# JoHof/lungmask

Hardware: NVIDIA H100
Metric: CT slices/sec @256x256 (R231) (higher is better)
Workload: dtype f16x3 (fp32-class: every fp32 value is an fp16 hi + scaled fp16 lo pair, 3 exact products per MAC, fp32 accumulate)

## Files before the change

lungmask_b200/csrc/conv_tc.cu:

```cuda
#include <atomic>
#include <stdio.h>
#include "conv_tc.cuh"
#include "sm90_ptx.cuh"

namespace lm {
namespace {

constexpr int BM = 128, BK = kBK, TILE_H = 16, TILE_W = 8;
constexpr int ROW_BYTES = 128;
constexpr int HALO_W = TILE_W + 2, HALO_H = TILE_H + 2;
constexpr int A_PLANE_BYTES_3x3 = HALO_W * HALO_H * ROW_BYTES;
constexpr int A_PLANE_BYTES_1x1 = BM * ROW_BYTES;
constexpr int A_BUF_BYTES = 2 * A_PLANE_BYTES_3x3;
constexpr int NUM_A_BUFS = 2;
constexpr int NUM_THREADS = 384;
constexpr int NUM_CONSUMER_WARPS = 8;
constexpr int MAX_CLASSES = 8;
constexpr int REGS_PRODUCER = 40, REGS_CONSUMER = 232;

template <int BN>
struct Cfg {
  static constexpr int B_PLANE_BYTES = BN * ROW_BYTES;
  static constexpr int STAGE_BYTES = 2 * B_PLANE_BYTES;
  static constexpr int STAGES = (BN == 64) ? 6 : 4;
  static constexpr int NUM_BARS = 2 * STAGES + 2 * NUM_A_BUFS;
  static constexpr int OFF_B = NUM_A_BUFS * A_BUF_BYTES;
  static constexpr int OFF_BARS = OFF_B + STAGES * STAGE_BYTES;
  static constexpr int OFF_HEAD = OFF_BARS + NUM_BARS * 8;
  static constexpr int DYN_SMEM = OFF_HEAD + ((BN == 64) ? (MAX_CLASSES * 64 + MAX_CLASSES) * 4 : 0);
  static_assert(DYN_SMEM <= 232448, "shared-memory budget (227 KB per CTA)");
};

struct TileCoord {
  int n, y0, x0, n0;
};

__device__ __forceinline__ TileCoord decode_tile(int tile, int n_tiles, int tiles_x, int tiles_img, int BN) {
  TileCoord t;
  const int mt = tile / n_tiles;
  t.n0 = (tile - mt * n_tiles) * BN;
  t.n = mt / tiles_img;
  const int r = mt - t.n * tiles_img;
  const int ty = r / tiles_x;
  t.y0 = ty * TILE_H;
  t.x0 = (r - ty * tiles_x) * TILE_W;
  return t;
}

template <int MC>
struct WorkItems {
  int first, step, total, n_tiles;
  uint32_t rank;
  __device__ WorkItems(int total_tiles, int n_tiles_) : n_tiles(n_tiles_) {
    rank = (MC > 1) ? cluster_ctarank() : 0u;
    first = (int)blockIdx.x / MC;
    step = (int)gridDim.x / MC;
    total = total_tiles / MC;
  }
  __device__ int tile(int item) const {
    if (MC == 1) return item;
    const int mtp = item / n_tiles;
    return (MC * mtp + (int)rank) * n_tiles + (item - mtp * n_tiles);
  }
};

__device__ __forceinline__ void store_split_pair(op_t* dst, size_t plane_stride, float a, float b) {
#if LM_OPERAND_F16
  uint32_t hi, lo;
  split_f16x2(a, b, hi, lo);
  *reinterpret_cast<uint32_t*>(dst) = hi;
  *reinterpret_cast<uint32_t*>(dst + plane_stride) = lo;
#else
  float ha, la, hb, lb;
  split_tf32(a, ha, la);
  split_tf32(b, hb, lb);
  *reinterpret_cast<float2*>(dst) = make_float2(ha, hb);
  *reinterpret_cast<float2*>(dst + plane_stride) = make_float2(la, lb);
#endif
}

__device__ __forceinline__ float2 ldg2_or_zero(const float* p, int c) {
  return p ? __ldg(reinterpret_cast<const float2*>(p + c)) : make_float2(0.f, 0.f);
}

template <int BN, int TAPS, int MC>
__device__ __forceinline__ void conv_consumer(const ConvParams& p, uint32_t smem_a, uint32_t smem_b, uint32_t full0,
                                              uint32_t empty0, uint32_t afull0, uint32_t aempty0, const float* s_head_w,
                                              const float* s_head_b) {
  using C = Cfg<BN>;
  constexpr int NA = BN / 2;
  constexpr int STAGES = C::STAGES;
  constexpr int PATCH_W = (TAPS == 9) ? HALO_W : TILE_W;
  constexpr uint32_t A_PLANE = (uint32_t)((TAPS == 9) ? A_PLANE_BYTES_3x3 : A_PLANE_BYTES_1x1);
  constexpr uint32_t SBO_A = PATCH_W * ROW_BYTES;
  const int tid = threadIdx.x - 128;
  const int half = tid >> 7, wq = (tid >> 5) & 3, lane = tid & 31;
  const int g = lane >> 2, qd = lane & 3;
  const int tiles_x = p.W / TILE_W, tiles_img = tiles_x * (p.H / TILE_H);
  const int n_tiles = p.Cout / BN;
  const int total_tiles = p.N * tiles_img * n_tiles;
  const int num_cb = (p.C0 + p.C1) / BK;
  const int num_kb = num_cb * TAPS, chunk_kb = p.chunk_kb;
  const uint32_t a_half = (uint32_t)(8 * half * PATCH_W * ROW_BYTES);

  const WorkItems<MC> items(total_tiles, n_tiles);
  float S[NA], P[NA], Q[NA];
  uint32_t s = 0, ph = 0, ab = 0, aph = 0;
  auto release = [&](uint32_t st, int a) {
    __syncwarp();
    if (lane == 0) {
      mbar_arrive(empty0 + 8 * st);
      if (MC > 1) mbar_arrive_cluster(empty0 + 8 * st, items.rank ^ 1u);
      if (a >= 0) mbar_arrive(aempty0 + 8 * a);
    }
  };
  auto mma_one = [&](float (&D)[NA], uint64_t da, uint64_t db, int acc) {
    if constexpr (BN == 128) wgmma_n128(D, da, db, acc); else wgmma_n64(D, da, db, acc);
  };

  for (int item = items.first; item < items.total; item += items.step) {
    const TileCoord t = decode_tile(items.tile(item), n_tiles, tiles_x, tiles_img, BN);
#pragma unroll
    for (int i = 0; i < NA; ++i) { S[i] = 0.f; Q[i] = 0.f; }
    for (int kb0 = 0; kb0 < num_kb; kb0 += chunk_kb) {
      const int kb1 = min(kb0 + chunk_kb, num_kb);
      uint32_t pend_s = 0;
      int pend_a = -1;
      for (int kb = kb0; kb < kb1; ++kb) {
        const int tap = (TAPS == 9) ? kb % 9 : 0;
        if (tap == 0) mbar_spin(afull0 + 8 * ab, aph);
        const uint32_t a_tap = smem_a + ab * (uint32_t)A_BUF_BYTES + a_half + (uint32_t)(((tap / 3) * PATCH_W + (tap % 3)) * ROW_BYTES);
        const uint32_t b_st = smem_b + s * (uint32_t)C::STAGE_BYTES;
        mbar_spin(full0 + 8 * s, ph);
        wgmma_fence();
#pragma unroll
        for (int k = 0; k < ROW_BYTES / 32; ++k) {
          const uint64_t ah = make_desc_sw128(a_tap + 32 * k, SBO_A), al = make_desc_sw128(a_tap + A_PLANE + 32 * k, SBO_A);
          const uint64_t bh = make_desc_sw128(b_st + 32 * k, 1024), bl = make_desc_sw128(b_st + C::B_PLANE_BYTES + 32 * k, 1024);
          mma_one(P, ah, bh, k != 0 || kb != kb0);
          mma_one(Q, ah, bl, 1);
          mma_one(Q, al, bh, 1);
        }
        wgmma_commit();
        if (kb > kb0) {
          wgmma_wait<1>();
          release(pend_s, pend_a);
        }
        pend_s = s;
        pend_a = (tap == TAPS - 1) ? (int)ab : -1;
        if (++s == STAGES) { s = 0; ph ^= 1u; }
        if (tap == TAPS - 1 && ++ab == NUM_A_BUFS) { ab = 0; aph ^= 1u; }
      }
      wgmma_wait<0>();
      release(pend_s, pend_a);
#pragma unroll
      for (int i = 0; i < NA; ++i) S[i] += P[i];
    }
#pragma unroll
    for (int i = 0; i < NA; ++i) S[i] += Q[i] * kLoUnscale;

    const float unscale = p.in_unscale;
    const int y = t.y0 + 8 * half + 2 * wq, x = t.x0 + g;
    const int c0 = t.n0 + 2 * qd;
    if (p.mode == kModeLinear) {
      float* out = static_cast<float*>(p.out);
#pragma unroll
      for (int j = 0; j < BN / 8; ++j) {
        const int c = c0 + 8 * j;
        const float2 b = ldg2_or_zero(p.bias, c);
#pragma unroll
        for (int r = 0; r < 2; ++r)
          *reinterpret_cast<float2*>(out + (((size_t)t.n * p.H + y + r) * p.W + x) * p.Cout + c) =
              make_float2(__fmaf_rn(S[4 * j + 2 * r], unscale, b.x), __fmaf_rn(S[4 * j + 2 * r + 1], unscale, b.y));
      }
      continue;
    }
    const float cscale = (p.mode == kModeHead) ? 1.f : p.out_scale;
#pragma unroll
    for (int j = 0; j < BN / 8; ++j) {
      const int c = c0 + 8 * j;
      const float2 b = ldg2_or_zero(p.bias, c), sc = ldg2_or_zero(p.scale, c), sh = ldg2_or_zero(p.shift, c);
      const float s0 = sc.x * cscale, s1 = sc.y * cscale, h0 = sh.x * cscale, h1 = sh.y * cscale;
#pragma unroll
      for (int r = 0; r < 2; ++r) {
        float& v0 = S[4 * j + 2 * r];
        float& v1 = S[4 * j + 2 * r + 1];
        v0 = __fadd_rn(__fmul_rn(fmaxf(__fmaf_rn(v0, unscale, b.x), 0.f), s0), h0);
        v1 = __fadd_rn(__fmul_rn(fmaxf(__fmaf_rn(v1, unscale, b.y), 0.f), s1), h1);
      }
    }
    if (BN == 64 && p.mode == kModeHead) {
      float lg[2][MAX_CLASSES];
#pragma unroll
      for (int k = 0; k < MAX_CLASSES; ++k) {
        float d0 = 0.f, d1 = 0.f;
        if (k < p.K) {
#pragma unroll
          for (int j = 0; j < BN / 8; ++j) {
#pragma unroll
            for (int e = 0; e < 2; ++e) {
              const float w = s_head_w[k * 64 + 8 * j + 2 * qd + e];
              d0 = fmaf(w, S[4 * j + e], d0);
              d1 = fmaf(w, S[4 * j + 2 + e], d1);
            }
          }
        }
        d0 += __shfl_xor_sync(0xffffffffu, d0, 1);
        d1 += __shfl_xor_sync(0xffffffffu, d1, 1);
        d0 += __shfl_xor_sync(0xffffffffu, d0, 2);
        d1 += __shfl_xor_sync(0xffffffffu, d1, 2);
        lg[0][k] = (k < p.K) ? d0 + s_head_b[k] : -INFINITY;
        lg[1][k] = (k < p.K) ? d1 + s_head_b[k] : -INFINITY;
      }
      if (qd == 0) {
#pragma unroll
        for (int r = 0; r < 2; ++r) {
          float mx = -INFINITY;
#pragma unroll
          for (int k = 0; k < MAX_CLASSES; ++k) mx = fmaxf(mx, lg[r][k]);
          float se = 0.f;
#pragma unroll
          for (int k = 0; k < MAX_CLASSES; ++k) if (k < p.K) se += expf(lg[r][k] - mx);
          const float lse = logf(se);
          int best = 0;
          float bestv = -INFINITY;
#pragma unroll
          for (int k = 0; k < MAX_CLASSES; ++k) {
            if (k < p.K) {
              const float sc = (lg[r][k] - mx) - lse;
              if (sc > bestv) { bestv = sc; best = k; }
              if (p.scores) p.scores[(((size_t)t.n * p.K + k) * p.H + y + r) * p.W + x] = sc;
            }
          }
          p.labels[((size_t)t.n * p.H + y + r) * p.W + x] = (uint8_t)best;
        }
      }
      continue;
    }
#if LM_OPERAND_F16
    {
      bool ovf = false;
#pragma unroll
      for (int i = 0; i < NA; ++i) ovf |= !(fabsf(S[i]) <= kOpMax);
      if (__any_sync(0xffffffffu, ovf) && lane == 0 && p.range_flag) *p.range_flag = 1;
    }
#endif
    {
      const size_t plane = (size_t)p.H * p.W * p.Cout;
      op_t* img = static_cast<op_t*>(p.out) + (size_t)t.n * 2 * plane;
#pragma unroll
      for (int j = 0; j < BN / 8; ++j)
#pragma unroll
        for (int r = 0; r < 2; ++r)
          store_split_pair(img + ((size_t)(y + r) * p.W + x) * p.Cout + c0 + 8 * j, plane, S[4 * j + 2 * r], S[4 * j + 2 * r + 1]);
    }
    if (p.mode == kModeReluBnPool) {
      const int Hp = p.H / 2, Wp = p.W / 2;
      const size_t plane = (size_t)Hp * Wp * p.Cout;
      op_t* img = static_cast<op_t*>(p.out_pool) + (size_t)t.n * 2 * plane + ((size_t)(y >> 1) * Wp + (x >> 1)) * p.Cout + c0;
#pragma unroll
      for (int j = 0; j < BN / 8; ++j) {
        float pv[2];
#pragma unroll
        for (int e = 0; e < 2; ++e) {
          const float top = S[4 * j + e] + __shfl_xor_sync(0xffffffffu, S[4 * j + e], 4);
          const float bot = S[4 * j + 2 + e] + __shfl_xor_sync(0xffffffffu, S[4 * j + 2 + e], 4);
          pv[e] = (top + bot) * 0.25f;
        }
        if ((g & 1) == 0) store_split_pair(img + 8 * j, plane, pv[0], pv[1]);
      }
    }
  }
}

template <int BN, int MC>
__global__ void __launch_bounds__(NUM_THREADS, 1)
conv_tc_kernel(const __grid_constant__ CUtensorMap tmA0, const __grid_constant__ CUtensorMap tmA1,
               const __grid_constant__ CUtensorMap tmB, const __grid_constant__ CUtensorMap tmBX, const ConvParams p) {
  using C = Cfg<BN>;
  constexpr int STAGES = C::STAGES;
  extern __shared__ __align__(1024) uint8_t smem[];
  uint64_t* bars = reinterpret_cast<uint64_t*>(smem + C::OFF_BARS);
  float* s_head_w = reinterpret_cast<float*>(smem + C::OFF_HEAD);
  float* s_head_b = s_head_w + MAX_CLASSES * 64;
  const uint32_t full0 = smem_u32(&bars[0]), empty0 = full0 + 8 * STAGES;
  const uint32_t afull0 = full0 + 16 * STAGES, aempty0 = afull0 + 8 * NUM_A_BUFS;
  const uint32_t smem_a = smem_u32(smem), smem_b = smem_a + C::OFF_B;
  const int warp = threadIdx.x >> 5;

  if (threadIdx.x == 0) {
    for (int s = 0; s < STAGES; ++s) { mbar_init(full0 + 8 * s, 1); mbar_init(empty0 + 8 * s, MC * NUM_CONSUMER_WARPS); }
    for (int s = 0; s < NUM_A_BUFS; ++s) { mbar_init(afull0 + 8 * s, 1); mbar_init(aempty0 + 8 * s, NUM_CONSUMER_WARPS); }
    fence_mbar_init();
    tma_prefetch_desc(&tmA0); tma_prefetch_desc(&tmA1); tma_prefetch_desc(MC > 1 ? &tmBX : &tmB);
  }
  if (BN == 64 && p.mode == kModeHead) {
    for (int i = threadIdx.x; i < p.K * 64; i += NUM_THREADS) s_head_w[i] = p.head_w[i];
    if (threadIdx.x < p.K) s_head_b[threadIdx.x] = p.head_b[threadIdx.x];
  }
  __syncthreads();
  if (MC > 1) cluster_sync_all();

  if (warp >= 4) {
    setmaxnreg_inc<REGS_CONSUMER>();
    if (p.taps == 9) conv_consumer<BN, 9, MC>(p, smem_a, smem_b, full0, empty0, afull0, aempty0, s_head_w, s_head_b);
    else conv_consumer<BN, 1, MC>(p, smem_a, smem_b, full0, empty0, afull0, aempty0, s_head_w, s_head_b);
  } else {
    setmaxnreg_dec<REGS_PRODUCER>();
    if (warp == 0) {
      const int tiles_x = p.W / TILE_W, tiles_img = tiles_x * (p.H / TILE_H);
      const int n_tiles = p.Cout / BN;
      const WorkItems<MC> items(p.N * tiles_img * n_tiles, n_tiles);
      const int taps = p.taps, halo = taps == 9 ? 1 : 0;
      const int num_cb = (p.C0 + p.C1) / BK;
      const uint32_t a_tx = 2u * (uint32_t)(taps == 9 ? A_PLANE_BYTES_3x3 : A_PLANE_BYTES_1x1);
      uint32_t s = 0, ph = 0, ab = 0, aph = 0;
      for (int item = items.first; item < items.total; item += items.step) {
        const TileCoord t = decode_tile(items.tile(item), n_tiles, tiles_x, tiles_img, BN);
        int c = 0;
        for (int cb = 0; cb < num_cb; ++cb, c += BK) {
          mbar_wait_inline(aempty0 + 8 * ab, aph ^ 1);
          if (elect_one()) {
            mbar_arrive_expect_tx(afull0 + 8 * ab, a_tx);
            const uint32_t dst = smem_a + ab * A_BUF_BYTES;
            if (c < p.C0) tma_load_5d(dst, &tmA0, afull0 + 8 * ab, c, t.x0 - halo, t.y0 - halo, 0, t.n);
            else          tma_load_5d(dst, &tmA1, afull0 + 8 * ab, c - p.C0, t.x0 - halo, t.y0 - halo, 0, t.n);
          }
          __syncwarp();
          if (++ab == NUM_A_BUFS) { ab = 0; aph ^= 1; }
          for (int tap = 0; tap < taps; ++tap) {
            mbar_wait_inline(empty0 + 8 * s, ph ^ 1);
            if (elect_one()) {
              mbar_arrive_expect_tx(full0 + 8 * s, C::STAGE_BYTES);
              if (MC > 1)
                tma_load_4d_mcast(smem_b + s * C::STAGE_BYTES + items.rank * (uint32_t)C::B_PLANE_BYTES, &tmBX, full0 + 8 * s, c, t.n0,
                                  tap, (int)items.rank, (uint16_t)((1u << MC) - 1u));
              else
                tma_load_4d(smem_b + s * C::STAGE_BYTES, &tmB, full0 + 8 * s, c, t.n0, tap, 0);
            }
            __syncwarp();
            if (++s == STAGES) { s = 0; ph ^= 1; }
          }
        }
      }
    }
  }
  if (MC > 1) cluster_sync_all();
}

typedef CUresult (*EncodeTiledFn)(CUtensorMap*, CUtensorMapDataType, cuuint32_t, void*, const cuuint64_t*,
                                  const cuuint64_t*, const cuuint32_t*, const cuuint32_t*,
                                  CUtensorMapInterleave, CUtensorMapSwizzle, CUtensorMapL2promotion,
                                  CUtensorMapFloatOOBfill);

EncodeTiledFn get_encode_fn() {
  static EncodeTiledFn fn = nullptr;
  if (!fn) {
    void* f = nullptr;
    cudaDriverEntryPointQueryResult qres;
    if (cudaGetDriverEntryPoint("cuTensorMapEncodeTiled", &f, cudaEnableDefault, &qres) != cudaSuccess) return nullptr;
    fn = reinterpret_cast<EncodeTiledFn>(f);
  }
  return fn;
}

#if LM_OPERAND_F16
constexpr CUtensorMapDataType kOpType = CU_TENSOR_MAP_DATA_TYPE_FLOAT16;
#else
constexpr CUtensorMapDataType kOpType = CU_TENSOR_MAP_DATA_TYPE_FLOAT32;
#endif

int encode(CUtensorMap* m, CUtensorMapDataType dtype, const void* base, int rank, const cuuint64_t* dims,
           const cuuint64_t* strides, const cuuint32_t* box) {
  EncodeTiledFn fn = get_encode_fn();
  if (!fn) return -1;
  cuuint32_t es[5] = {1, 1, 1, 1, 1};
  CUresult r = fn(m, dtype, (cuuint32_t)rank, const_cast<void*>(base), dims, strides, box,
                  es, CU_TENSOR_MAP_INTERLEAVE_NONE, CU_TENSOR_MAP_SWIZZLE_128B,
                  CU_TENSOR_MAP_L2_PROMOTION_L2_256B, CU_TENSOR_MAP_FLOAT_OOB_FILL_NONE);
  return r == CUDA_SUCCESS ? 0 : (int)r;
}

int make_act_map(CUtensorMap* m, const void* base, int n_cap, int H, int W, int Cch, int taps) {
  const cuuint64_t E = kOpBytes;
  cuuint64_t dims[5] = {(cuuint64_t)Cch, (cuuint64_t)W, (cuuint64_t)H, 2, (cuuint64_t)n_cap};
  cuuint64_t strides[4] = {(cuuint64_t)Cch * E, (cuuint64_t)W * Cch * E, (cuuint64_t)H * W * Cch * E,
                           (cuuint64_t)2 * H * W * Cch * E};
  const cuuint32_t halo = taps == 9 ? 2 : 0;
  cuuint32_t box[5] = {BK, TILE_W + halo, TILE_H + halo, 2, 1};
  return encode(m, kOpType, base, 5, dims, strides, box);
}

}

int make_conv_maps(ConvMaps* maps, const void* src0, const void* src1, const void* weights,
                   const ConvParams& p, int n_capacity) {
  const cuuint64_t E = kOpBytes;
  if (p.H % TILE_H || p.W % TILE_W || p.C0 % BK || p.C1 % BK || (p.taps != 1 && p.taps != 9)) return -2;
  const int BN = conv_tile_n(p);
  if (p.Cout % BN) return -3;
  int r = make_act_map(&maps->a0, src0, n_capacity, p.H, p.W, p.C0, p.taps);
  if (r) return r;
  r = (p.C1 > 0) ? make_act_map(&maps->a1, src1, n_capacity, p.H, p.W, p.C1, p.taps)
                 : make_act_map(&maps->a1, src0, n_capacity, p.H, p.W, p.C0, p.taps);
  if (r) return r;
  const int Cin = p.C0 + p.C1;
  cuuint64_t dims[4] = {(cuuint64_t)Cin, (cuuint64_t)p.Cout, (cuuint64_t)p.taps, 2};
  cuuint64_t strides[3] = {(cuuint64_t)Cin * E, (cuuint64_t)p.Cout * Cin * E, (cuuint64_t)p.taps * p.Cout * Cin * E};
  cuuint32_t box[4] = {BK, (cuuint32_t)BN, 1, 2}, box_x[4] = {BK, (cuuint32_t)BN, 1, 1};
  r = encode(&maps->b, kOpType, weights, 4, dims, strides, box);
  return r ? r : encode(&maps->bx, kOpType, weights, 4, dims, strides, box_x);
}


template <int BN, int MC>
static int launch_impl(const ConvMaps& maps, const ConvParams& p, int num_sms, cudaStream_t stream) {
  static std::atomic<unsigned long long> attr_set_mask{0ull};
  int dev = 0;
  if (cudaGetDevice(&dev) != cudaSuccess || dev < 0 || dev >= 64) return -9;
  if (!((attr_set_mask.load(std::memory_order_acquire) >> dev) & 1ull)) {
    cudaError_t e = cudaFuncSetAttribute(conv_tc_kernel<BN, MC>, cudaFuncAttributeMaxDynamicSharedMemorySize, Cfg<BN>::DYN_SMEM);
    if (e != cudaSuccess) return (int)e;
    attr_set_mask.fetch_or(1ull << dev, std::memory_order_release);
  }
  const int total = p.N * (p.H / TILE_H) * (p.W / TILE_W) * (p.Cout / BN);
  const int groups = total / MC, sm_groups = num_sms / MC;
  cudaLaunchConfig_t cfg = {};
  cfg.gridDim = dim3((unsigned)(MC * (groups < sm_groups ? groups : sm_groups)), 1, 1);
  cfg.blockDim = dim3(NUM_THREADS, 1, 1);
  cfg.dynamicSmemBytes = Cfg<BN>::DYN_SMEM;
  cfg.stream = stream;
  cudaLaunchAttribute attr[1];
  attr[0].id = cudaLaunchAttributeClusterDimension;
  attr[0].val.clusterDim.x = MC; attr[0].val.clusterDim.y = 1; attr[0].val.clusterDim.z = 1;
  cfg.attrs = attr;
  cfg.numAttrs = 1;
  cudaError_t e = cudaLaunchKernelEx(&cfg, conv_tc_kernel<BN, MC>, maps.a0, maps.a1, maps.b, maps.bx, p);
  return (int)(e != cudaSuccess ? e : cudaGetLastError());
}

int conv_tc_prepare() {
  cudaError_t e = cudaFuncSetAttribute(conv_tc_kernel<128, 1>, cudaFuncAttributeMaxDynamicSharedMemorySize, Cfg<128>::DYN_SMEM);
  if (e == cudaSuccess) e = cudaFuncSetAttribute(conv_tc_kernel<64, 1>, cudaFuncAttributeMaxDynamicSharedMemorySize, Cfg<64>::DYN_SMEM);
  if (e == cudaSuccess) e = cudaFuncSetAttribute(conv_tc_kernel<128, 2>, cudaFuncAttributeMaxDynamicSharedMemorySize, Cfg<128>::DYN_SMEM);
  if (e == cudaSuccess) e = cudaFuncSetAttribute(conv_tc_kernel<64, 2>, cudaFuncAttributeMaxDynamicSharedMemorySize, Cfg<64>::DYN_SMEM);
  return (int)e;
}

int launch_conv_tc(const ConvMaps& maps, const ConvParams& p, int num_sms, cudaStream_t stream) {
  if (p.mode == kModeHead && (p.Cout != 64 || p.K > MAX_CLASSES)) return -4;
  if (p.chunk_kb < 1) return -5;
  if (p.weight_mcast == 2)
    return conv_tile_n(p) == 128 ? launch_impl<128, 2>(maps, p, num_sms, stream) : launch_impl<64, 2>(maps, p, num_sms, stream);
  return conv_tile_n(p) == 128 ? launch_impl<128, 1>(maps, p, num_sms, stream) : launch_impl<64, 1>(maps, p, num_sms, stream);
}

}
```

Before: 1392.

## Overlap next tile's first WGMMAs with epilogue; vectorize stores via quad transpose

The consumer now issues the first one or two k-blocks of the next tile's MMAs before running the current tile's epilogue, so tensor-core work overlaps the epilogue's stores and arithmetic. This uses extra accumulator registers (P2 for BN=64), and the release and fold bookkeeping becomes more intricate. Epilogue stores are also regrouped with an intra-quad shuffle transpose so each thread writes 16-byte vectors instead of 4- or 8-byte pieces, cutting store instruction count at the cost of extra shuffles. Head-mode BN=64 and 1x1 layers keep the old path.

New measurement: 1473 (median of 6 runs). 1.06x the previous value.

```diff
diff --git a/lungmask_b200/csrc/conv_tc.cu b/lungmask_b200/csrc/conv_tc.cu
--- a/lungmask_b200/csrc/conv_tc.cu
+++ b/lungmask_b200/csrc/conv_tc.cu
@@ -64,18 +64,57 @@
   }
 };
 
-__device__ __forceinline__ void store_split_pair(op_t* dst, size_t plane_stride, float a, float b) {
+__device__ __forceinline__ void quad_transpose(uint32_t (&x)[4], int qd) {
+#pragma unroll
+  for (int m = 2; m >= 1; m >>= 1) {
+    const bool up = (qd & m) != 0;
+#pragma unroll
+    for (int k = 0; k < 4; ++k) {
+      if (k & m) continue;
+      const uint32_t recv = __shfl_xor_sync(0xffffffffu, up ? x[k] : x[k ^ m], m);
+      x[k] = up ? recv : x[k];
+      x[k ^ m] = up ? x[k ^ m] : recv;
+    }
+  }
+}
+__device__ __forceinline__ void quad_transpose(float2 (&v)[4], int qd) {
+  uint32_t a[4], b[4];
+#pragma unroll
+  for (int k = 0; k < 4; ++k) { a[k] = __float_as_uint(v[k].x); b[k] = __float_as_uint(v[k].y); }
+  quad_transpose(a, qd);
+  quad_transpose(b, qd);
+#pragma unroll
+  for (int k = 0; k < 4; ++k) v[k] = make_float2(__uint_as_float(a[k]), __uint_as_float(b[k]));
+}
+
+__device__ __forceinline__ void store_split8(op_t* dst, size_t plane_stride, const float2 (&v)[4], int qd, bool pred) {
 #if LM_OPERAND_F16
-  uint32_t hi, lo;
-  split_f16x2(a, b, hi, lo);
-  *reinterpret_cast<uint32_t*>(dst) = hi;
-  *reinterpret_cast<uint32_t*>(dst + plane_stride) = lo;
+  uint32_t hi[4], lo[4];
+#pragma unroll
+  for (int k = 0; k < 4; ++k) split_f16x2(v[k].x, v[k].y, hi[k], lo[k]);
+  quad_transpose(hi, qd);
+  quad_transpose(lo, qd);
+  if (pred) {
+    *reinterpret_cast<uint4*>(dst) = make_uint4(hi[0], hi[1], hi[2], hi[3]);
+    *reinterpret_cast<uint4*>(dst + plane_stride) = make_uint4(lo[0], lo[1], lo[2], lo[3]);
+  }
 #else
-  float ha, la, hb, lb;
-  split_tf32(a, ha, la);
-  split_tf32(b, hb, lb);
-  *reinterpret_cast<float2*>(dst) = make_float2(ha, hb);
-  *reinterpret_cast<float2*>(dst + plane_stride) = make_float2(la, lb);
+  float2 h[4], l[4];
+#pragma unroll
+  for (int k = 0; k < 4; ++k) {
+    split_tf32(v[k].x, h[k].x, l[k].x);
+    split_tf32(v[k].y, h[k].y, l[k].y);
+  }
+  quad_transpose(h, qd);
+  quad_transpose(l, qd);
+  if (pred) {
+    float4* dh = reinterpret_cast<float4*>(dst);
+    float4* dl = reinterpret_cast<float4*>(dst + plane_stride);
+    dh[0] = make_float4(h[0].x, h[0].y, h[1].x, h[1].y);
+    dh[1] = make_float4(h[2].x, h[2].y, h[3].x, h[3].y);
+    dl[0] = make_float4(l[0].x, l[0].y, l[1].x, l[1].y);
+    dl[1] = make_float4(l[2].x, l[2].y, l[3].x, l[3].y);
+  }
 #endif
 }
 
@@ -83,7 +122,7 @@
   return p ? __ldg(reinterpret_cast<const float2*>(p + c)) : make_float2(0.f, 0.f);
 }
 
-template <int BN, int TAPS, int MC>
+template <int BN, int TAPS, int MC, bool LOOKAHEAD>
 __device__ __forceinline__ void conv_consumer(const ConvParams& p, uint32_t smem_a, uint32_t smem_b, uint32_t full0,
                                               uint32_t empty0, uint32_t afull0, uint32_t aempty0, const float* s_head_w,
                                               const float* s_head_b) {
@@ -102,9 +141,14 @@
   const int num_cb = (p.C0 + p.C1) / BK;
   const int num_kb = num_cb * TAPS, chunk_kb = p.chunk_kb;
   const uint32_t a_half = (uint32_t)(8 * half * PATCH_W * ROW_BYTES);
+  static_assert(!LOOKAHEAD || TAPS == 9, "look-ahead: 3x3 layers only");
+  const int la = !LOOKAHEAD ? 0 : (BN == 64 || chunk_kb >= 2) ? 2 : 1;
+  const bool la_split = BN == 64 && chunk_kb == 1 && la == 2;
+  const bool la_fold = la > 0 && (la_split || la % chunk_kb == 0 || la == num_kb);
 
   const WorkItems<MC> items(total_tiles, n_tiles);
   float S[NA], P[NA], Q[NA];
+  float P2[(BN == 64) ? NA : 1];
   uint32_t s = 0, ph = 0, ab = 0, aph = 0;
   auto release = [&](uint32_t st, int a) {
     __syncwarp();
@@ -117,61 +161,115 @@
   auto mma_one = [&](float (&D)[NA], uint64_t da, uint64_t db, int acc) {
     if constexpr (BN == 128) wgmma_n128(D, da, db, acc); else wgmma_n64(D, da, db, acc);
   };
-
-  for (int item = items.first; item < items.total; item += items.step) {
-    const TileCoord t = decode_tile(items.tile(item), n_tiles, tiles_x, tiles_img, BN);
-#pragma unroll
-    for (int i = 0; i < NA; ++i) { S[i] = 0.f; Q[i] = 0.f; }
-    for (int kb0 = 0; kb0 < num_kb; kb0 += chunk_kb) {
-      const int kb1 = min(kb0 + chunk_kb, num_kb);
+  auto issue_kb = [&](float (&D)[NA], int kb, bool hh_restart) -> int {
+    const int tap = (TAPS == 9) ? kb % 9 : 0;
+    if (tap == 0) mbar_spin(afull0 + 8 * ab, aph);
+    const uint32_t a_tap = smem_a + ab * (uint32_t)A_BUF_BYTES + a_half + (uint32_t)(((tap / 3) * PATCH_W + (tap % 3)) * ROW_BYTES);
+    const uint32_t b_st = smem_b + s * (uint32_t)C::STAGE_BYTES;
+    mbar_spin(full0 + 8 * s, ph);
+    wgmma_fence();
+#pragma unroll
+    for (int k = 0; k < ROW_BYTES / 32; ++k) {
+      const uint64_t ah = make_desc_sw128(a_tap + 32 * k, SBO_A), al = make_desc_sw128(a_tap + A_PLANE + 32 * k, SBO_A);
+      const uint64_t bh = make_desc_sw128(b_st + 32 * k, 1024), bl = make_desc_sw128(b_st + C::B_PLANE_BYTES + 32 * k, 1024);
+      mma_one(D, ah, bh, k != 0 || !hh_restart);
+      mma_one(Q, ah, bl, 1);
+      mma_one(Q, al, bh, 1);
+    }
+    wgmma_commit();
+    const int a = (tap == TAPS - 1) ? (int)ab : -1;
+    if (++s == STAGES) { s = 0; ph ^= 1u; }
+    if (tap == TAPS - 1 && ++ab == NUM_A_BUFS) { ab = 0; aph ^= 1u; }
+    return a;
+  };
+  uint32_t la_s = 0;
+  auto issue_lookahead = [&]() {
+    if constexpr (LOOKAHEAD) {
+#pragma unroll
+      for (int i = 0; i < NA; ++i) Q[i] = 0.f;
+      la_s = s;
+      issue_kb(P, 0, true);
+      if (la_split) {
+        if constexpr (BN == 64) issue_kb(P2, 1, true);
+      } else if (la > 1) {
+        issue_kb(P, 1, false);
+      }
+    }
+  };
+
+  int item = items.first;
+  if (item < items.total) issue_lookahead();
+  for (; item < items.total; item += items.step) {
+    wgmma_wait<0>();
+    if constexpr (LOOKAHEAD) {
+      release(la_s, -1);
+      if (la > 1) release(la_s + 1 == STAGES ? 0 : la_s + 1, -1);
+    } else {
+#pragma unroll
+      for (int i = 0; i < NA; ++i) Q[i] = 0.f;
+    }
+#pragma unroll
+    for (int i = 0; i < NA; ++i) S[i] = 0.f;
+    if (la_fold) {
+#pragma unroll
+      for (int i = 0; i < NA; ++i) S[i] += P[i];
+      if constexpr (BN == 64) {
+        if (la_split) {
+#pragma unroll
+          for (int i = 0; i < NA; ++i) S[i] += P2[i];
+        }
+      }
+    }
+    for (int kb0 = la; kb0 < num_kb;) {
+      const int kb1 = min((kb0 / chunk_kb + 1) * chunk_kb, num_kb);
+      const bool restart = kb0 % chunk_kb == 0;
       uint32_t pend_s = 0;
       int pend_a = -1;
       for (int kb = kb0; kb < kb1; ++kb) {
-        const int tap = (TAPS == 9) ? kb % 9 : 0;
-        if (tap == 0) mbar_spin(afull0 + 8 * ab, aph);
-        const uint32_t a_tap = smem_a + ab * (uint32_t)A_BUF_BYTES + a_half + (uint32_t)(((tap / 3) * PATCH_W + (tap % 3)) * ROW_BYTES);
-        const uint32_t b_st = smem_b + s * (uint32_t)C::STAGE_BYTES;
-        mbar_spin(full0 + 8 * s, ph);
-        wgmma_fence();
-#pragma unroll
-        for (int k = 0; k < ROW_BYTES / 32; ++k) {
-          const uint64_t ah = make_desc_sw128(a_tap + 32 * k, SBO_A), al = make_desc_sw128(a_tap + A_PLANE + 32 * k, SBO_A);
-          const uint64_t bh = make_desc_sw128(b_st + 32 * k, 1024), bl = make_desc_sw128(b_st + C::B_PLANE_BYTES + 32 * k, 1024);
-          mma_one(P, ah, bh, k != 0 || kb != kb0);
-          mma_one(Q, ah, bl, 1);
-          mma_one(Q, al, bh, 1);
-        }
-        wgmma_commit();
+        const uint32_t st = s;
+        const int a = issue_kb(P, kb, restart && kb == kb0);
         if (kb > kb0) {
           wgmma_wait<1>();
           release(pend_s, pend_a);
         }
-        pend_s = s;
-        pend_a = (tap == TAPS - 1) ? (int)ab : -1;
-        if (++s == STAGES) { s = 0; ph ^= 1u; }
-        if (tap == TAPS - 1 && ++ab == NUM_A_BUFS) { ab = 0; aph ^= 1u; }
+        pend_s = st;
+        pend_a = a;
       }
       wgmma_wait<0>();
       release(pend_s, pend_a);
 #pragma unroll
       for (int i = 0; i < NA; ++i) S[i] += P[i];
+      kb0 = kb1;
     }
 #pragma unroll
     for (int i = 0; i < NA; ++i) S[i] += Q[i] * kLoUnscale;
 
+    if (item + items.step < items.total) issue_lookahead();
+    const TileCoord tc = decode_tile(items.tile(item), n_tiles, tiles_x, tiles_img, BN);
+
     const float unscale = p.in_unscale;
-    const int y = t.y0 + 8 * half + 2 * wq, x = t.x0 + g;
-    const int c0 = t.n0 + 2 * qd;
+    const int y = tc.y0 + 8 * half + 2 * wq, x = tc.x0 + g;
+    const int c0 = tc.n0 + 2 * qd;
     if (p.mode == kModeLinear) {
-      float* out = static_cast<float*>(p.out);
-#pragma unroll
-      for (int j = 0; j < BN / 8; ++j) {
-        const int c = c0 + 8 * j;
-        const float2 b = ldg2_or_zero(p.bias, c);
-#pragma unroll
-        for (int r = 0; r < 2; ++r)
-          *reinterpret_cast<float2*>(out + (((size_t)t.n * p.H + y + r) * p.W + x) * p.Cout + c) =
-              make_float2(__fmaf_rn(S[4 * j + 2 * r], unscale, b.x), __fmaf_rn(S[4 * j + 2 * r + 1], unscale, b.y));
+      float* out = static_cast<float*>(p.out) + ((size_t)tc.n * p.H * p.W + x) * p.Cout + tc.n0 + 8 * qd;
+#pragma unroll
+      for (int m = 0; m < BN / 32; ++m) {
+        float2 b[4];
+#pragma unroll
+        for (int k = 0; k < 4; ++k) b[k] = ldg2_or_zero(p.bias, c0 + 8 * (4 * m + k));
+#pragma unroll
+        for (int r = 0; r < 2; ++r) {
+          float2 v[4];
+#pragma unroll
+          for (int k = 0; k < 4; ++k) {
+            const int j = 4 * m + k;
+            v[k] = make_float2(__fmaf_rn(S[4 * j + 2 * r], unscale, b[k].x), __fmaf_rn(S[4 * j + 2 * r + 1], unscale, b[k].y));
+          }
+          quad_transpose(v, qd);
+          float4* dst = reinterpret_cast<float4*>(out + (size_t)(y + r) * p.W * p.Cout + 32 * m);
+          dst[0] = make_float4(v[0].x, v[0].y, v[1].x, v[1].y);
+          dst[1] = make_float4(v[2].x, v[2].y, v[3].x, v[3].y);
+        }
       }
       continue;
     }
@@ -229,10 +327,10 @@
             if (k < p.K) {
               const float sc = (lg[r][k] - mx) - lse;
               if (sc > bestv) { bestv = sc; best = k; }
-              if (p.scores) p.scores[(((size_t)t.n * p.K + k) * p.H + y + r) * p.W + x] = sc;
+              if (p.scores) p.scores[(((size_t)tc.n * p.K + k) * p.H + y + r) * p.W + x] = sc;
             }
           }
-          p.labels[((size_t)t.n * p.H + y + r) * p.W + x] = (uint8_t)best;
+          p.labels[((size_t)tc.n * p.H + y + r) * p.W + x] = (uint8_t)best;
         }
       }
       continue;
@@ -247,30 +345,41 @@
 #endif
     {
       const size_t plane = (size_t)p.H * p.W * p.Cout;
-      op_t* img = static_cast<op_t*>(p.out) + (size_t)t.n * 2 * plane;
-#pragma unroll
-      for (int j = 0; j < BN / 8; ++j)
-#pragma unroll
-        for (int r = 0; r < 2; ++r)
-          store_split_pair(img + ((size_t)(y + r) * p.W + x) * p.Cout + c0 + 8 * j, plane, S[4 * j + 2 * r], S[4 * j + 2 * r + 1]);
+      op_t* img = static_cast<op_t*>(p.out) + (size_t)tc.n * 2 * plane + ((size_t)y * p.W + x) * p.Cout + tc.n0 + 8 * qd;
+#pragma unroll
+      for (int m = 0; m < BN / 32; ++m)
+#pragma unroll
+        for (int r = 0; r < 2; ++r) {
+          float2 v[4];
+#pragma unroll
+          for (int k = 0; k < 4; ++k) v[k] = make_float2(S[4 * (4 * m + k) + 2 * r], S[4 * (4 * m + k) + 2 * r + 1]);
+          store_split8(img + (size_t)r * p.W * p.Cout + 32 * m, plane, v, qd, true);
+        }
     }
     if (p.mode == kModeReluBnPool) {
       const int Hp = p.H / 2, Wp = p.W / 2;
       const size_t plane = (size_t)Hp * Wp * p.Cout;
-      op_t* img = static_cast<op_t*>(p.out_pool) + (size_t)t.n * 2 * plane + ((size_t)(y >> 1) * Wp + (x >> 1)) * p.Cout + c0;
-#pragma unroll
-      for (int j = 0; j < BN / 8; ++j) {
-        float pv[2];
-#pragma unroll
-        for (int e = 0; e < 2; ++e) {
-          const float top = S[4 * j + e] + __shfl_xor_sync(0xffffffffu, S[4 * j + e], 4);
-          const float bot = S[4 * j + 2 + e] + __shfl_xor_sync(0xffffffffu, S[4 * j + 2 + e], 4);
-          pv[e] = (top + bot) * 0.25f;
-        }
-        if ((g & 1) == 0) store_split_pair(img + 8 * j, plane, pv[0], pv[1]);
-      }
-    }
-  }
+      op_t* img = static_cast<op_t*>(p.out_pool) + (size_t)tc.n * 2 * plane + ((size_t)(y >> 1) * Wp + (x >> 1)) * p.Cout + tc.n0 + 8 * qd;
+#pragma unroll
+      for (int m = 0; m < BN / 32; ++m) {
+        float2 v[4];
+#pragma unroll
+        for (int k = 0; k < 4; ++k) {
+          const int j = 4 * m + k;
+          float pv[2];
+#pragma unroll
+          for (int e = 0; e < 2; ++e) {
+            const float top = S[4 * j + e] + __shfl_xor_sync(0xffffffffu, S[4 * j + e], 4);
+            const float bot = S[4 * j + 2 + e] + __shfl_xor_sync(0xffffffffu, S[4 * j + 2 + e], 4);
+            pv[e] = (top + bot) * 0.25f;
+          }
+          v[k] = make_float2(pv[0], pv[1]);
+        }
+        store_split8(img + 32 * m, plane, v, qd, (g & 1) == 0);
+      }
+    }
+  }
+  wgmma_wait<0>();
 }
 
 template <int BN, int MC>
@@ -303,8 +412,10 @@
 
   if (warp >= 4) {
     setmaxnreg_inc<REGS_CONSUMER>();
-    if (p.taps == 9) conv_consumer<BN, 9, MC>(p, smem_a, smem_b, full0, empty0, afull0, aempty0, s_head_w, s_head_b);
-    else conv_consumer<BN, 1, MC>(p, smem_a, smem_b, full0, empty0, afull0, aempty0, s_head_w, s_head_b);
+    if (p.taps == 9 && !(BN == 64 && p.mode == kModeHead))
+      conv_consumer<BN, 9, MC, true>(p, smem_a, smem_b, full0, empty0, afull0, aempty0, s_head_w, s_head_b);
+    else if (p.taps == 9) conv_consumer<BN, 9, MC, false>(p, smem_a, smem_b, full0, empty0, afull0, aempty0, s_head_w, s_head_b);
+    else conv_consumer<BN, 1, MC, false>(p, smem_a, smem_b, full0, empty0, afull0, aempty0, s_head_w, s_head_b);
   } else {
     setmaxnreg_dec<REGS_PRODUCER>();
     if (warp == 0) {
```
